# robotvisionmu/DenseMonoSLAM

Measured on AMD Instinct MI355X. Metric: frames/sec ICP+RGB+fusion @640x480, higher is better.
Workload: dtype f32; 1 GPU; TUM fr1/desk-like 640x480 full 3-level ICP+RGB tracking (SO3 + {10,5,4} GN iterations) + surfel index-map fusion; synthetic box-room RGB-D stream, loop closure off (--o), NID keyframing off (--nkf); cameras_per_gpu=1, n_pred=2, n_pred_project_passes=1, surfels_per_map=246557, surfels_total=246557, exchange=none (1 camera)

## Files before the change

densemonoslam_amd/csrc/exact_arith.hpp:

```cpp
#pragma once
#include <hip/hip_runtime.h>

namespace dms {
namespace exact {

struct Divisor {
  float d, y;
};

__device__ __forceinline__ Divisor divisor(float d) { return Divisor{d, 1.0f / d}; }

__device__ __forceinline__ float div(float a, const Divisor& c) {
  float q = a * c.y;
  float r = __builtin_fmaf(-c.d, q, a);
  q = __builtin_fmaf(r, c.y, q);
  r = __builtin_fmaf(-c.d, q, a);
  return __builtin_fmaf(r, c.y, q);
}

__device__ __forceinline__ float sqrt_normal(float a) {
  const float s = __builtin_amdgcn_sqrtf(a);
  const float sd = __uint_as_float(__float_as_uint(s) - 1u), su = __uint_as_float(__float_as_uint(s) + 1u);
  const float ed = __builtin_fmaf(-sd, s, a), eu = __builtin_fmaf(-su, s, a);
  float o = ed <= 0.f ? sd : s;
  o = eu > 0.f ? su : o;
  return o;
}

__device__ __forceinline__ float rcp_1_4(float s) {
  const float y0 = __builtin_amdgcn_rcpf(s);
  const float e = __builtin_fmaf(-s, y0, 1.0f);
  return __builtin_fmaf(e, y0, y0);
}

__device__ __forceinline__ Divisor divisor_1_4(float s) { return Divisor{s, rcp_1_4(s)}; }

}
}
```

densemonoslam_amd/csrc/fusion_fuse.hip:

```cpp
#include "scan.hpp"
#include "smallmath.hpp"
#include <utility>

#include "surfel.hpp"

namespace dms {

struct FuseArgs {
  const dms_pose_block* pose;
  const uchar4* rgba;
  const float* dr;
  const float* drf;
  const unsigned* index;
  const float4* vertConf;
  const float4* normRad;
  int cols, rows, slot_h;
  float cx, cy, icx, icy;
  float maxDepth, timef, weighting;
  const float* weighting_dev;
  int time, timeIdx;
  int transposed;
  int xcd;
};

__device__ __forceinline__ f3 dv_vertex(const float* depth, int cols, int sx, int sy, float x, float y, float cx, float cy, float icx,
                                        float icy) {
  const float z = depth[(size_t)sy * cols + sx];
  return mk3(((x - cx) * z) * icx, ((y - cy) * z) * icy, z);
}

__device__ __forceinline__ f3 dv_normal(const float* depth, int cols, int rows, const f3& vPosition, float tx, float ty, float x, float y,
                                        float cx, float cy, float icx, float icy) {
  const float colsf = (float)cols, rowsf = (float)rows;
  const int sx = texel(tx, colsf, cols), sy = texel(ty, rowsf, rows);
  const int sxf = texel(tx + (1.0f / colsf), colsf, cols), sxb = texel(tx - (1.0f / colsf), colsf, cols);
  const int syf = texel(ty + (1.0f / rowsf), rowsf, rows), syb = texel(ty - (1.0f / rowsf), rowsf, rows);
  const f3 xf = dv_vertex(depth, cols, sxf, sy, x + 1.f, y, cx, cy, icx, icy);
  const f3 xb = dv_vertex(depth, cols, sxb, sy, x - 1.f, y, cx, cy, icx, icy);
  const f3 yf = dv_vertex(depth, cols, sx, syf, x, y + 1.f, cx, cy, icx, icy);
  const f3 yb = dv_vertex(depth, cols, sx, syb, x, y - 1.f, cx, cy, icx, icy);
  const f3 del_x = mk3(((xb.x + vPosition.x) / 2.f) - ((xf.x + vPosition.x) / 2.f), ((xb.y + vPosition.y) / 2.f) - ((xf.y + vPosition.y) / 2.f),
                       ((xb.z + vPosition.z) / 2.f) - ((xf.z + vPosition.z) / 2.f));
  const f3 del_y = mk3(((yb.x + vPosition.x) / 2.f) - ((yf.x + vPosition.x) / 2.f), ((yb.y + vPosition.y) / 2.f) - ((yf.y + vPosition.y) / 2.f),
                       ((yb.z + vPosition.z) / 2.f) - ((yf.z + vPosition.z) / 2.f));
  return normalized3(cross3(del_x, del_y));
}

__device__ __forceinline__ float angle_between(const f3& a, const f3& b) {
  return det_acosf(dot3(a, b) / (length3(a) * length3(b)));
}

__global__ __launch_bounds__(256) void k_fuse_associate(FuseArgs a, float4* __restrict__ slot_pos, float4* __restrict__ slot_col,
                                                        float4* __restrict__ slot_nrm, unsigned* __restrict__ slot_best,
                                                        unsigned char* __restrict__ slot_flag, unsigned* __restrict__ winner, int slot_w) {
  const int tiles_j = (a.slot_h + 7) >> 3;
  const int t = xcd_block(blockIdx.x, gridDim.x, a.xcd) * (blockDim.x >> 6) + (threadIdx.x >> 6);
  const int ti = t / tiles_j, tj = t - ti * tiles_j;
  const int lane = threadIdx.x & 63, quad = lane >> 2, sub = lane & 3;
  const int i = ti * 2 + (quad >> 3);
  const int j = tj * 8 + (quad & 7);
  if (i >= slot_w || j >= a.slot_h) return;
  const int slot = i * a.slot_h + j;
  const int par = ((a.time % 2) + 2) % 2;
  const int px = 2 * i + par, py = 2 * j + par;
  unsigned char flag = 0;
  if (px < a.cols && py < a.rows) {
    const float colsf = (float)a.cols, rowsf = (float)a.rows;
    const float tx = uv_coord(px, a.cols), ty = uv_coord(py, a.rows);
    const float x = tx * colsf, y = ty * rowsf;
    const int sx = texel(tx, colsf, a.cols), sy = texel(ty, rowsf, a.rows);
    const f3 vPosLocal = dv_vertex(a.dr, a.cols, sx, sy, x, y, a.cx, a.cy, a.icx, a.icy);
    bool ok = ((int)x % 2 == (int)a.timef % 2) && ((int)y % 2 == (int)a.timef % 2);
    if (ok) {
      const int sxb = texel(tx - (1.0f / colsf), colsf, a.cols), sxf = texel(tx + (1.0f / colsf), colsf, a.cols);
      const int syb = texel(ty - (1.0f / rowsf), rowsf, a.rows), syf = texel(ty + (1.0f / rowsf), rowsf, a.rows);
      ok = !(a.dr[(size_t)sy * a.cols + sxb] == 0.f) && !(a.dr[(size_t)syb * a.cols + sx] == 0.f) &&
           !(a.dr[(size_t)sy * a.cols + sxf] == 0.f) && !(a.dr[(size_t)syf * a.cols + sx] == 0.f);
    }
    ok = ok && vPosLocal.z > 0.f && vPosLocal.z <= a.maxDepth;
    const float weighting = a.weighting_dev ? *a.weighting_dev : a.weighting;
    ok = ok && !(weighting < 0.f);
    if (ok) {
      const float* P = a.pose->pose;
      const f3 vPos = xform_point(P, vPosLocal);
      const f3 vPos_f = dv_vertex(a.drf, a.cols, sx, sy, x, y, a.cx, a.cy, a.icx, a.icy);
      const uchar4 c = a.rgba[(size_t)sy * a.cols + sx];
      const f3 vNormLocal = dv_normal(a.drf, a.cols, a.rows, vPos_f, tx, ty, x, y, a.cx, a.cy, a.icx, a.icy);
      const f3 nG = xform_dir(P, vNormLocal);
      const float rad = surfel_radius(vPos_f.z, vNormLocal.z, a.icx, a.icy);
      const float conf = surfel_confidence(x, y, a.cx, a.cy, weighting);

      int counter = 0;
      unsigned best = 0u;
      const float scale = 1.0f;
      const float indexXStep = (1.0f / (colsf * scale)) * 0.5f;
      const float indexYStep = (1.0f / (rowsf * scale)) * 0.5f;
      float bestDist = 1000.f;
      const float windowMultiplier = 2.f;
      const float xl = (x - a.cx) * a.icx;
      const float yl = (y - a.cy) * a.icy;
      const float lambda = sqrtf((xl * xl + yl * yl) + 1.f);
      const f3 ray = mk3(xl, yl, 1.f);
      const float ray_len = length3(ray);
      const float x_lo = tx - ((scale * indexXStep) * windowMultiplier), x_hi = tx + ((scale * indexXStep) * windowMultiplier);
      const float y_lo = ty - ((scale * indexYStep) * windowMultiplier), y_hi = ty + ((scale * indexYStep) * windowMultiplier);
      const AxisTaps tx_ = axis_taps(x_lo, x_hi, indexXStep, colsf, a.cols);
      const AxisTaps ty_ = axis_taps(y_lo, y_hi, indexYStep, rowsf, a.rows);
      const int txs_s = sub == 0 ? tx_.t0 : sub == 1 ? tx_.t1 : sub == 2 ? tx_.t2 : tx_.t3;
      const int mxs_s = sub == 0 ? tx_.m0 : sub == 1 ? tx_.m1 : sub == 2 ? tx_.m2 : tx_.m3;
      const int tys[4] = {ty_.t0, ty_.t1, ty_.t2, ty_.t3}, mys[4] = {ty_.m0, ty_.m1, ty_.m2, ty_.m3};
      size_t q[4];
      bool used[4];
      unsigned cur[4];
      float4 vcs[4], nrs[4];
#pragma unroll
      for (int jj = 0; jj < 4; ++jj) {
        const bool u = mxs_s != 0 && mys[jj] != 0;
        const int ux = u ? txs_s : 0, uy = u ? tys[jj] : 0;
        used[jj] = u;
        q[jj] = a.transposed ? (size_t)ux * a.rows + uy : (size_t)uy * a.cols + ux;
      }
#pragma unroll
      for (int jj = 0; jj < 4; ++jj) {
        cur[jj] = a.index[q[jj]];
        vcs[jj] = a.vertConf[q[jj]];
        nrs[jj] = a.normRad[q[jj]];
      }
      int order = 64;
#pragma unroll
      for (int jj = 0; jj < 4; ++jj) {
        const unsigned current = cur[jj];
        if (used[jj] && current > 0u) {
          const float4 vc = vcs[jj];
          if (fabsf((vc.z * lambda) - (vPosLocal.z * lambda)) < 0.05f) {
            const float dist = length3(cross3(ray, mk3(vc.x, vc.y, vc.z))) / ray_len;
            const float4 nr = nrs[jj];
            if (dist < bestDist && (fabsf(nr.z) < 0.75f || fabsf(angle_between(mk3(nr.x, nr.y, nr.z), vNormLocal)) < 0.5f)) {
              counter++;
              bestDist = dist;
              best = current;
              order = sub * 4 + jj;
            }
          }
        }
      }
#pragma unroll
      for (int m = 1; m < 4; m <<= 1) {
        const float od = __shfl_xor(bestDist, m, 64);
        const int oo = __shfl_xor(order, m, 64);
        const unsigned ob = __shfl_xor(best, m, 64);
        counter += __shfl_xor(counter, m, 64);
        if (od < bestDist || (od == bestDist && oo < order)) {
          bestDist = od;
          order = oo;
          best = ob;
        }
      }
      flag = counter > 0 ? 1 : 2;
      if (sub == 0) {
        slot_pos[slot] = make_float4(vPos.x, vPos.y, vPos.z, conf);
        slot_col[slot] = make_float4(encode_color_bytes(c.x, c.y, c.z), 0.f, a.timef, flag == 1 ? -1.f : -2.f);
        slot_nrm[slot] = make_float4(nG.x, nG.y, nG.z, rad);
        slot_best[slot] = best;
        if (flag == 1) atomicMin(winner + best, (unsigned)slot);
      }
    }
  }
  if (sub == 0) slot_flag[slot] = flag;
}

__global__ __launch_bounds__(256) void k_fuse_update(int nslots, const float4* __restrict__ slot_pos, const float4* __restrict__ slot_col,
                                                     const float4* __restrict__ slot_nrm, const unsigned* __restrict__ slot_best,
                                                     const unsigned char* __restrict__ slot_flag, unsigned* __restrict__ winner,
                                                     SurfelPlanes sp, size_t cap, int time, int timeIdx) {
  const int slot = blockIdx.x * blockDim.x + threadIdx.x;
  if (slot >= nslots || slot_flag[slot] != 1) return;
  const unsigned id = slot_best[slot];
  if (winner[id] != (unsigned)slot) return;
  winner[id] = kEmptyWinner;
  fuse_update_apply(id, (unsigned)slot, slot_pos, slot_col, slot_nrm, sp, cap, time, timeIdx);
}

struct CleanArgs {
  const dms_pose_block* pose;
  const unsigned* index;
  const float4* vertConf;
  const float4* colorTime;
  const float* depth_synth;
  int cols, rows;
  float cx, cy, fx, fy;
  float confThreshold, maxDepth;
  int time, timeIdx, timeDelta, isFern;
  int nodes;
  const float* node_table;
  int nslots;
  int transposed;
  int suffix;
  int num_sensors;
  int planes;
};

struct F4 {
  float x, y, z, w;
};
__device__ __forceinline__ F4 ld4(const float4* p) {
  const float4 t = *p;
  F4 r;
  r.x = t.x;
  r.y = t.y;
  r.z = t.z;
  r.w = t.w;
  return r;
}
__device__ __forceinline__ float4 to4(const F4& v) { return make_float4(v.x, v.y, v.z, v.w); }
struct CleanElem {
  F4 pos, col, nrm;
  float times[DMS_MAX_SENSORS];
  float vt;
};

__device__ __forceinline__ bool clean_load(unsigned e, unsigned M, const SurfelPlanes& sp, size_t cap, const float4* slot_pos,
                                           const float4* slot_col, const float4* slot_nrm, const unsigned char* slot_flag, int nslots,
                                           int timeIdx, int planes, CleanElem& o) {
  if (e < M) {
    o.pos = ld4(sp.pos + e);
    o.col = ld4(sp.col + e);
    o.nrm = ld4(sp.nrm + e);
#pragma unroll
    for (int s = 0; s < DMS_MAX_SENSORS; ++s) o.times[s] = s < planes ? sp.times[(size_t)s * cap + e] : -3.f;
    o.vt = sp.times[(size_t)timeIdx * cap + e];
    return true;
  }
  const unsigned slot = e - M;
  if ((int)slot >= nslots || slot_flag[slot] == 0) return false;
  o.pos = ld4(slot_pos + slot);
  o.col = ld4(slot_col + slot);
  o.nrm = ld4(slot_nrm + slot);
#pragma unroll
  for (int s = 0; s < DMS_MAX_SENSORS; ++s) o.times[s] = (s == timeIdx) ? o.col.w : -3.f;
  o.vt = o.col.w;
  return true;
}

__device__ __forceinline__ int clean_test(const CleanArgs& a, const CleanElem& v) {
  int test = 1;
  const float* Tinv = a.pose->t_inv;
  const f3 localPos = xform_point(Tinv, mk3(v.pos.x, v.pos.y, v.pos.z));
  const float x = ((a.fx * localPos.x) / localPos.z) + a.cx;
  const float y = ((a.fy * localPos.y) / localPos.z) + a.cy;
  const f3 localNorm = normalized3(xform_dir(Tinv, mk3(v.nrm.x, v.nrm.y, v.nrm.z)));
  const float colsf = (float)a.cols, rowsf = (float)a.rows;
  const float scale = 1.0f;
  const float indexXStep = (1.0f / (colsf * scale)) * 0.5f;
  const float indexYStep = (1.0f / (rowsf * scale)) * 0.5f;
  const float windowMultiplier = 2.f;
  int count = 0, zCount = 0;
  const float vt = v.vt;
  if ((float)a.time - vt < (float)a.timeDelta && localPos.z > 0.f && x > 0.f && y > 0.f && x < colsf && y < rowsf) {
    const float xc = x / colsf, yc = y / rowsf;
    const float x_lo = xc - ((scale * indexXStep) * windowMultiplier), x_hi = xc + ((scale * indexXStep) * windowMultiplier);
    const float y_lo = yc - ((scale * indexYStep) * windowMultiplier), y_hi = yc + ((scale * indexYStep) * windowMultiplier);
    const AxisTaps tx_ = axis_taps(x_lo, x_hi, indexXStep, colsf, a.cols);
    const AxisTaps ty_ = axis_taps(y_lo, y_hi, indexYStep, rowsf, a.rows);
    const int txs[4] = {tx_.t0, tx_.t1, tx_.t2, tx_.t3}, mxs[4] = {tx_.m0, tx_.m1, tx_.m2, tx_.m3};
    const int tys[4] = {ty_.t0, ty_.t1, ty_.t2, ty_.t3}, mys[4] = {ty_.m0, ty_.m1, ty_.m2, ty_.m3};
#pragma unroll
    for (int i = 0; i < 4; ++i) {
      if (mxs[i] != 0) {
        float4 vcs[4];
        unsigned qs[4];
        int mult[4];
#pragma unroll
        for (int j = 0; j < 4; ++j) {
          mult[j] = mxs[i] * mys[j];
          const int uy = mult[j] ? tys[j] : 0;
          qs[j] = a.transposed ? (unsigned)txs[i] * (unsigned)a.rows + (unsigned)uy : (unsigned)uy * (unsigned)a.cols + (unsigned)txs[i];
          vcs[j] = a.vertConf[qs[j]];
        }
#pragma unroll
        for (int j = 0; j < 4; ++j) {
          const int m = mult[j];
          const float4 vc = vcs[j];
          if (m != 0 && vc.w > a.confThreshold && vc.z > localPos.z) {
            const unsigned cur = a.index[qs[j]];
            const float2 ct = *reinterpret_cast<const float2*>(reinterpret_cast<const float*>(&a.colorTime[qs[j]]) + 2);
            if (cur > 0u) {
              const float ctz = ct.x, ctw = ct.y;
              const float dx = vc.x - localPos.x, dy = vc.y - localPos.y;
              if (ctz < v.col.z && vc.z - localPos.z < 0.01f && sqrtf(dx * dx + dy * dy) < v.nrm.w * 1.4f) count += m;
              if (ctw == (float)a.time && vc.z - localPos.z > 0.01f && fabsf(localNorm.z) > 0.85f) zCount += m;
            }
          }
        }
      }
    }
  }
  if (count > 8 || zCount > 4) test = 0;
  const float vt2 = (vt == -2.f) ? (float)a.time : vt;
  int unHealthy = 0;
#pragma unroll
  for (int s = 0; s < DMS_MAX_SENSORS; ++s) {
    const float ts = (s == a.timeIdx) ? vt2 : v.times[s];
    if (s < a.num_sensors && (ts == -1.f || (((float)a.time - ts) > 20.f && v.pos.w < a.confThreshold))) unHealthy++;
  }
  if (unHealthy == a.num_sensors) test = 0;
  if (vt2 > 0.f && (float)a.time - vt2 > (float)a.timeDelta) test = 1;
  return test;
}

__global__ __launch_bounds__(256) void k_clean_flags(CleanArgs a, SurfelPlanes sp, size_t cap, const unsigned* __restrict__ d_count,
                                                     const float4* slot_pos, const float4* slot_col, const float4* slot_nrm,
                                                     const unsigned char* slot_flag, unsigned char* __restrict__ keep,
                                                     unsigned* __restrict__ block_count, unsigned* __restrict__ first_touched) {
  const unsigned M = d_count[0];
  const unsigned total = M + (unsigned)a.nslots;
  const unsigned base = blockIdx.x * kScanChunk;
  if (first_touched && blockIdx.x == 0 && threadIdx.x == 0) *first_touched = 0xFFFFFFFFu;
  unsigned cnt = 0;
  if (base < total) {
    for (int k = 0; k < kScanChunk / 256; ++k) {
      const unsigned e = base + k * 256 + threadIdx.x;
      unsigned char f = 0;
      if (e < total) {
        CleanElem v;
        if (a.suffix && e < M) {
          v.pos = ld4(sp.pos + e);
#pragma unroll
          for (int s = 0; s < DMS_MAX_SENSORS; ++s) v.times[s] = s < a.planes ? sp.times[(size_t)s * cap + e] : -3.f;
          v.vt = sp.times[(size_t)a.timeIdx * cap + e];
          const f3 lp = xform_point(a.pose->t_inv, mk3(v.pos.x, v.pos.y, v.pos.z));
          const float x = ((a.fx * lp.x) / lp.z) + a.cx, y = ((a.fy * lp.y) / lp.z) + a.cy;
          const bool windowed = (float)a.time - v.vt < (float)a.timeDelta && lp.z > 0.f && x > 0.f && y > 0.f && x < (float)a.cols &&
                                y < (float)a.rows;
          const F4 zero = {0.f, 0.f, 0.f, 0.f};
          v.col = windowed ? ld4(sp.col + e) : zero;
          v.nrm = windowed ? ld4(sp.nrm + e) : zero;
          f = (unsigned char)clean_test(a, v);
        } else if (clean_load(e, M, sp, cap, slot_pos, slot_col, slot_nrm, slot_flag, a.nslots, a.timeIdx, a.planes, v)) {
          f = (unsigned char)clean_test(a, v);
        }
        keep[e] = f;
      }
      cnt += f;
    }
  }
  const unsigned tot = block_sum_u32(cnt);
  if (threadIdx.x == 0) block_count[blockIdx.x] = tot;
}

__device__ __forceinline__ f3 node_pos(const float* nt, int j) { return mk3(nt[j * 16 + 0], nt[j * 16 + 1], nt[j * 16 + 2]); }
// ... 209 lines not shown
          v.col.w = (float)a.time;
          v.vt = (float)a.time;
        }
        out.pos[dst] = to4(v.pos);
        out.col[dst] = to4(v.col);
        out.nrm[dst] = to4(v.nrm);
#pragma unroll
        for (int s = 0; s < DMS_MAX_SENSORS; ++s)
          if (s < a.planes) out.times[(size_t)s * cap + dst] = (s == a.timeIdx) ? v.vt : v.times[s];
      }
    }
    if (e >= M && e < total) slot_flag[e - M] = 0;
  }
}

static bool dense_img(const dms_image2d& im, size_t elem, int w, int h) {
  return im.data && im.cols == w && im.rows == h && im.pitch == (size_t)w * elem;
}

int model_fuse(dms_model* m, const dms_pose_block* pose, int time, int timeIdx, const dms_image2d* rgba, const dms_image2d* dr,
               const dms_image2d* drf, const dms_indexmap_out* im, const dms_camera* cam, float depthCutoff, float weighting,
               const float* weighting_dev, int transposed, hipStream_t s, int defer_update) {
  DMS_REQUIRE(m && pose && rgba && dr && drf && im && cam, "null argument");
  DMS_REQUIRE(!m->pending_update, "a deferred update pass is still pending (index_map applies it)");
  DMS_REQUIRE(timeIdx >= 0 && timeIdx < DMS_MAX_SENSORS, "timeIdx out of range");
  if (m->live_planes < timeIdx + 1) m->live_planes = timeIdx + 1;
  const int W = m->width, H = m->height;
  DMS_REQUIRE(dense_img(*rgba, 4, W, H) && dense_img(*dr, 4, W, H) && dense_img(*drf, 4, W, H) && dense_img(im->index, 4, W, H) &&
                  dense_img(im->vertConf, 16, W, H) && dense_img(im->normRad, 16, W, H),
              "dense W×H images required");
  FuseArgs a;
  a.xcd = xcd_remap_enabled();
  a.pose = pose;
  a.rgba = (const uchar4*)rgba->data;
  a.dr = (const float*)dr->data;
  a.drf = (const float*)drf->data;
  a.index = (const unsigned*)im->index.data;
  a.vertConf = (const float4*)im->vertConf.data;
  a.normRad = (const float4*)im->normRad.data;
  a.cols = W;
  a.rows = H;
  a.slot_h = m->slot_h;
  a.cx = cam->cx;
  a.cy = cam->cy;
  a.icx = (float)(1.0 / (double)cam->fx);
  a.icy = (float)(1.0 / (double)cam->fy);
  a.maxDepth = depthCutoff;
  a.timef = (float)time;
  a.weighting = weighting;
  a.weighting_dev = weighting_dev;
  a.time = time;
  a.timeIdx = timeIdx;
  a.transposed = transposed ? 1 : 0;
  const int slot_w = (W + 1) / 2;
  const int tiles = ((m->slot_h + 7) / 8) * ((slot_w + 1) / 2);
  dim3 b(256), g((tiles + 3) / 4);
  hipLaunchKernelGGL(k_fuse_associate, g, b, 0, s, a, m->slot_pos, m->slot_col, m->slot_nrm, m->slot_best, m->slot_flag, m->winner, slot_w);
  DMS_CHECK_LAUNCH();
  if (defer_update) {
    m->pending_update = true;
    m->pending_time = time;
    m->pending_timeIdx = timeIdx;
  } else {
    hipLaunchKernelGGL(k_fuse_update, dim3((m->slots + 255) / 256), dim3(256), 0, s, m->slots, m->slot_pos, m->slot_col, m->slot_nrm,
                       m->slot_best, m->slot_flag, m->winner, m->buf[m->cur], m->cap, time, timeIdx);
    DMS_CHECK_LAUNCH();
  }
  m->version += 1;
  return DMS_OK;
}

int model_flush_pending(dms_model* m, hipStream_t s) {
  if (!m || !m->pending_update) return DMS_OK;
  m->pending_update = false;
  hipLaunchKernelGGL(k_fuse_update, dim3((m->slots + 255) / 256), dim3(256), 0, s, m->slots, m->slot_pos, m->slot_col, m->slot_nrm, m->slot_best,
                     m->slot_flag, m->winner, m->buf[m->cur], m->cap, m->pending_time, m->pending_timeIdx);
  DMS_CHECK_LAUNCH();
  return DMS_OK;
}

int model_clean(dms_model* m, const dms_pose_block* pose, int time, int timeIdx, const dms_indexmap_out* im, const dms_image2d* depth_synth,
                const dms_camera* cam, float confThreshold, const float* graph_host, int graph_nodes, int timeDelta, float maxDepth,
                int isFern, int transposed, unsigned* count_out2, hipStream_t s) {
  DMS_REQUIRE(m && !m->pending_update, "a deferred update pass is still pending (index_map applies it)");
  DMS_REQUIRE(m && pose && im && cam, "null argument");
  DMS_REQUIRE(timeIdx >= 0 && timeIdx < DMS_MAX_SENSORS, "timeIdx out of range");
  const int W = m->width, H = m->height;
  DMS_REQUIRE(dense_img(im->index, 4, W, H) && dense_img(im->vertConf, 16, W, H) && dense_img(im->colorTime, 16, W, H),
              "dense W×H index-map images required");
  if (graph_nodes >= m->max_nodes) {
    set_error("dms_model_clean: %d deformation nodes exceed the limit %d", graph_nodes, m->max_nodes);
    return DMS_ERR_CAPACITY;
  }
  if (graph_nodes > 0) {
    DMS_REQUIRE(graph_host, "null graph");
    DMS_HIP(hipMemcpyAsync(m->nodes, graph_host, (size_t)graph_nodes * 16 * sizeof(float), hipMemcpyHostToDevice, s));
  }
  CleanArgs a;
  a.pose = pose;
  a.index = (const unsigned*)im->index.data;
  a.vertConf = (const float4*)im->vertConf.data;
  a.colorTime = (const float4*)im->colorTime.data;
  a.depth_synth = (depth_synth && depth_synth->data) ? (const float*)depth_synth->data : nullptr;
  a.cols = W;
  a.rows = H;
  a.cx = cam->cx;
  a.cy = cam->cy;
  a.fx = cam->fx;
  a.fy = cam->fy;
  a.confThreshold = confThreshold;
  a.maxDepth = maxDepth;
  a.time = time;
  a.timeIdx = timeIdx;
  a.timeDelta = timeDelta;
  a.isFern = isFern;
  a.nodes = graph_nodes;
  a.node_table = m->nodes;
  a.nslots = m->slots;
  a.transposed = transposed ? 1 : 0;
  const size_t upper = m->count_upper + (size_t)m->slots;
  const int nb = (int)((upper + kScanChunk - 1) / kScanChunk);
  const bool suffix = graph_nodes == 0 && upper >= m->clean_suffix_min;
  a.suffix = suffix ? 1 : 0;
  a.num_sensors = m->num_sensors;
  if (m->live_planes < timeIdx + 1) m->live_planes = timeIdx + 1;
  static const bool all_planes = getenv("DMS_CLEAN_ALL_PLANES") != nullptr;
  a.planes = all_planes ? DMS_MAX_SENSORS : m->live_planes;
  const SurfelPlanes src = m->buf[m->cur], dst = m->buf[m->cur ^ 1];
  hipLaunchKernelGGL(k_clean_flags, dim3(nb), dim3(256), 0, s, a, src, m->cap, m->d_count, m->slot_pos, m->slot_col, m->slot_nrm,
                     m->slot_flag, m->keep, m->block_count, suffix ? m->clean_first : (unsigned*)nullptr);
  DMS_CHECK_LAUNCH();
  static const int inline_max = getenv("DMS_CLEAN_INLINE_SCAN_MAX") ? atoi(getenv("DMS_CLEAN_INLINE_SCAN_MAX")) : 2048;
  const bool inline_scan = nb <= inline_max && !suffix;
  if (!inline_scan) {
    hipLaunchKernelGGL(k_scan_blocks_par, dim3((nb + 1023) / 1024), dim3(1024), 0, s, m->block_count, m->block_offset, nb, m->d_count_alt,
                       (unsigned)m->cap, count_out2, suffix ? m->clean_first : (unsigned*)nullptr, m->d_count, (unsigned)kScanChunk);
    DMS_CHECK_LAUNCH();
  }
  const int suffix_grid = nb < 2048 ? nb : 2048;
  if (suffix)
    hipLaunchKernelGGL(k_clean_scatter_suffix, dim3(suffix_grid), dim3(256), 0, s, a, src, m->cap, m->d_count, m->slot_pos, m->slot_col,
                       m->slot_nrm, m->slot_flag, m->keep, m->block_offset, dst, m->clean_first);
  else
    hipLaunchKernelGGL(k_clean_scatter, dim3(nb), dim3(256), 0, s, a, src, m->cap, m->d_count, m->slot_pos, m->slot_col, m->slot_nrm,
                       m->slot_flag, m->keep, m->block_offset, dst, inline_scan ? m->block_count : (const unsigned*)nullptr, m->d_count_alt,
                       count_out2);
  DMS_CHECK_LAUNCH();
  if (suffix) {
    hipLaunchKernelGGL(k_clean_copy_back, dim3(suffix_grid), dim3(256), 0, s, dst, src, m->cap, m->d_count_alt, m->clean_first, a.planes);
    DMS_CHECK_LAUNCH();
  }
  std::swap(m->d_count, m->d_count_alt);
  if (!suffix) m->cur ^= 1;
  m->count_upper = upper < m->cap ? upper : m->cap;
  m->version += 1;
  return DMS_OK;
}

}
```

densemonoslam_amd/csrc/fusion_map.hip:

```cpp
#include <vector>

#include "exact_arith.hpp"
#include "scan.hpp"
#include "smallmath.hpp"
#include "surfel.hpp"
#include "fill.hpp"
#include "internal.hpp"
#include "track_init.hpp"

namespace dms {
int model_flush_pending(dms_model* m, hipStream_t s);

static size_t up256(size_t v) { return (v + 255) / 256 * 256; }

struct ModelCarver {
  char* base = nullptr;
  size_t off = 0;
  template <typename T>
  T* take(size_t n) {
    off = up256(off);
    T* p = base ? (T*)(base + off) : nullptr;
    off += n * sizeof(T);
    return p;
  }
// ... 8 lines not shown
  }
  m->d_count = c.take<unsigned>(8);
  m->d_count_alt = m->d_count ? m->d_count + 4 : nullptr;
  m->slot_pos = c.take<float4>(m->slots);
  m->slot_col = c.take<float4>(m->slots);
  m->slot_nrm = c.take<float4>(m->slots);
  m->slot_best = c.take<unsigned>(m->slots);
  m->slot_flag = c.take<unsigned char>(m->slots);
  m->winner = c.take<unsigned>(m->cap);
  const size_t total = m->cap + (size_t)m->width * m->height;
  m->keep = c.take<unsigned char>(total);
  m->block_count = c.take<unsigned>(total / kScanChunk + 2);
  m->block_offset = c.take<unsigned>(total / kScanChunk + 2);
  m->clean_first = c.take<unsigned>(4);
  m->nodes = c.take<float>((size_t)m->max_nodes * 16);
}

__global__ void k_fill_u32(unsigned* p, size_t n, unsigned v) {
  for (size_t i = blockIdx.x * (size_t)blockDim.x + threadIdx.x; i < n; i += (size_t)blockDim.x * gridDim.x) p[i] = v;
}

}

using namespace dms;

extern "C" {

int dms_model_create(dms_model** out, size_t capacity, int width, int height) {
  DMS_REQUIRE(out && width >= 16 && height >= 16, "bad argument");
  dms_model* m = new dms_model();
  m->cap = capacity ? capacity : (size_t)5700 * 5700;
  m->width = width;
  m->height = height;
  m->slot_h = (height + 1) / 2;
  m->slots = ((width + 1) / 2) * m->slot_h;
  ModelCarver sz;
  model_layout(m, sz);
  m->arena_bytes = up256(sz.off);
  hipError_t e = hipMalloc((void**)&m->arena, m->arena_bytes);
  if (e != hipSuccess) {
    delete m;
    return hip_fail(e, "hipMalloc(model)", __FILE__, __LINE__);
  }
  ModelCarver c;
  c.base = m->arena;
  model_layout(m, c);
  e = hipHostMalloc((void**)&m->h_count, 8 * sizeof(unsigned), hipHostMallocDefault);
  if (e != hipSuccess) {
    (void)hipFree(m->arena);
    delete m;
    return hip_fail(e, "hipHostMalloc", __FILE__, __LINE__);
  }
  DMS_HIP(hipMemset(m->d_count, 0, 8 * sizeof(unsigned)));
  hipLaunchKernelGGL(k_fill_u32, dim3(1024), dim3(256), 0, 0, m->winner, m->cap, kEmptyWinner);
  DMS_CHECK_LAUNCH();
  for (int b = 0; b < 2; ++b) {
    hipLaunchKernelGGL(k_fill_u32, dim3(2048), dim3(256), 0, 0, (unsigned*)m->buf[b].times, m->cap * DMS_MAX_SENSORS, 0xC0400000u);
    DMS_CHECK_LAUNCH();
  }
  DMS_HIP(hipDeviceSynchronize());
  m->count_upper = 0;
  if (const char* smin = getenv("DMS_CLEAN_SUFFIX_MIN")) m->clean_suffix_min = (size_t)atoll(smin);
  *out = m;
  return DMS_OK;
}

int dms_model_set_num_sensors(dms_model* m, int num_sensors) {
  DMS_REQUIRE(m, "null argument");
  DMS_REQUIRE(num_sensors >= 1 && num_sensors <= DMS_MAX_SENSORS, "num_sensors out of range");
  m->num_sensors = num_sensors;
  return DMS_OK;
}

int dms_model_set_clean_suffix_min(dms_model* m, size_t surfels) {
  DMS_REQUIRE(m, "null argument");
  m->clean_suffix_min = surfels;
  return DMS_OK;
}

int dms_model_destroy(dms_model* m) {
  if (!m) return DMS_OK;
  if (m->arena) (void)hipFree(m->arena);
  if (m->h_count) (void)hipHostFree(m->h_count);
  delete m;
  return DMS_OK;
}

size_t dms_model_capacity(dms_model* m) { return m ? m->cap : 0; }
size_t dms_model_count_bound(dms_model* m) { return m ? m->count_upper : 0; }

int dms_model_count(dms_model* m, unsigned int* count, dms_stream s) {
  DMS_REQUIRE(m && count, "null argument");
  DMS_HIP(hipMemcpyAsync(m->h_count, m->d_count, sizeof(unsigned), hipMemcpyDeviceToHost, (hipStream_t)s));
  DMS_HIP(hipStreamSynchronize((hipStream_t)s));
  *count = m->h_count[0];
  m->count_upper = *count;
  return DMS_OK;
}

static int model_download_planes(dms_model* m, unsigned n, std::vector<float4>& pos, std::vector<float4>& col, std::vector<float4>& nrm,
                                 std::vector<float>& times, hipStream_t s) {
  const SurfelPlanes& b = m->buf[m->cur];
  pos.resize(n);
  col.resize(n);
  nrm.resize(n);
  times.resize((size_t)n * DMS_MAX_SENSORS);
// ... 1044 lines not shown
```

densemonoslam_amd/csrc/selftest.hip:

```cpp
#include "exact_arith.hpp"
#include "internal.hpp"

namespace dms {

template <int WHAT>
__global__ __launch_bounds__(256) void k_exact_check(unsigned first, unsigned long long n, float d, unsigned long long* __restrict__ bad,
                                                     unsigned* __restrict__ first_bad) {
  const unsigned long long t = (unsigned long long)blockIdx.x * blockDim.x + threadIdx.x;
  const exact::Divisor c = exact::divisor(d);
  unsigned long long mine = 0;
  unsigned which = 0;
  for (unsigned long long i = t * 256ull; i < t * 256ull + 256ull && i < n; ++i) {
    const unsigned bits = first + (unsigned)i;
    const float a = __uint_as_float(bits);
    float want, got;
    if (WHAT == 0) {
      want = sqrtf(a);
      got = exact::sqrt_normal(a);
    } else if (WHAT == 1) {
      want = 1.0f / a;
      got = exact::rcp_1_4(a);
    } else {
      if (!(fabsf(a) <= 3.4028234e38f)) continue;
      if (a != 0.f && fabsf(a) < 1.2621774e-29f) continue;
      want = a / d;
      if (a != 0.f && !(fabsf(want) >= 1.2621774e-29f && fabsf(want) <= 3.4028234e38f)) continue;
      got = exact::div(a, c);
      if (want == 0.f && got == 0.f) continue;
    }
    if (__float_as_uint(want) != __float_as_uint(got)) {
      mine += 1;
      which = bits;
    }
  }
  if (mine) {
    atomicAdd(bad, mine);
    atomicMax(first_bad, which);
  }
}

}

using namespace dms;

extern "C" int dms_exact_arith_selftest(int what, float d, unsigned long long* mismatches, unsigned* first_bad) {
  DMS_REQUIRE(mismatches && what >= 0 && what <= 2, "bad argument");
  DMS_REQUIRE(what != 2 || (d == d && fabsf(d) >= 1.17549435e-38f && fabsf(d) <= 3.4028234e38f), "the divisor must be a normal number");
  unsigned first = 0;
  unsigned long long n = 0;
  if (what == 0) {
    first = 0x0F800000u;
    n = 0x7F800000ull - first;
  } else if (what == 1) {
    first = 0x3F800000u;
    n = 0x40800000ull - first;
  } else {
    first = 0u;
    n = 1ull << 32;
  }
  unsigned long long* d_bad = nullptr;
  DMS_HIP(hipMalloc((void**)&d_bad, 16));
  DMS_HIP(hipMemset(d_bad, 0, 16));
  unsigned* d_first = (unsigned*)(d_bad + 1);
  const unsigned long long threads = (n + 255ull) / 256ull;
  const unsigned blocks = (unsigned)((threads + 255ull) / 256ull);
  if (what == 0)
    hipLaunchKernelGGL(k_exact_check<0>, dim3(blocks), dim3(256), 0, 0, first, n, d, d_bad, d_first);
  else if (what == 1)
    hipLaunchKernelGGL(k_exact_check<1>, dim3(blocks), dim3(256), 0, 0, first, n, d, d_bad, d_first);
  else
    hipLaunchKernelGGL(k_exact_check<2>, dim3(blocks), dim3(256), 0, 0, first, n, d, d_bad, d_first);
  hipError_t e = hipGetLastError();
  unsigned long long host[2] = {0, 0};
  if (e == hipSuccess) e = hipMemcpy(host, d_bad, 16, hipMemcpyDeviceToHost);
  (void)hipFree(d_bad);
  if (e != hipSuccess) return hip_fail(e, "exact-arithmetic self-test", __FILE__, __LINE__);
  *mismatches = host[0];
  if (first_bad) *first_bad = (unsigned)host[1];
  return DMS_OK;
}
```

densemonoslam_amd/csrc/surfel.hpp:

```cpp
#pragma once
#include "common.hpp"
#include "detmath.hpp"
#include "../../include/dmslam_fusion.h"

namespace dms {

struct SurfelPlanes {
  float4* pos;
  float4* col;
  float4* nrm;
  float* times;
};

constexpr unsigned kEmptyWinner = 0xFFFFFFFFu;
constexpr unsigned long long kZClear = (0xFFFFFFull << 32) | 0xFFFFFFFFull;
constexpr int kScanChunk = 256;

__host__ __device__ __forceinline__ int texel(float u, float n_f, int n) {
  int i = (int)floorf(u * n_f);
  if (i < 0) i = 0;
  if (i > n - 1) i = n - 1;
  return i;
}
__host__ __device__ __forceinline__ unsigned depth24(float zw) {
  if (!(zw >= 0.f)) return 0xFFFFFFFFu;
  if (zw > 1.f) return 0xFFFFFFFFu;
  return (unsigned)(int)rint((double)zw * 16777215.0);
}

__host__ __device__ __forceinline__ f3 xform_point(const float* M, const f3& p) {
  return mk3(((M[0] * p.x + M[1] * p.y) + M[2] * p.z) + M[3], ((M[4] * p.x + M[5] * p.y) + M[6] * p.z) + M[7],
             ((M[8] * p.x + M[9] * p.y) + M[10] * p.z) + M[11]);
}
__host__ __device__ __forceinline__ f3 xform_dir(const float* M, const f3& v) {
  return mk3((M[0] * v.x + M[1] * v.y) + M[2] * v.z, (M[4] * v.x + M[5] * v.y) + M[6] * v.z,
             (M[8] * v.x + M[9] * v.y) + M[10] * v.z);
}
__host__ __device__ __forceinline__ float length3(const f3& a) { return sqrtf(dot3(a, a)); }

__host__ __device__ __forceinline__ float surfel_radius(float depth, float norm_z, float cam_z, float cam_w) {
  const float meanFocal = ((1.0f / fabsf(cam_z)) + (1.0f / fabsf(cam_w))) / 2.0f;
  const float sqrt2 = 1.41421356237f;
  const float radius = (depth / meanFocal) * sqrt2;
  float radius_n = radius;
  radius_n = radius_n / fabsf(norm_z);
  radius_n = fminf(2.0f * radius, radius_n);
  return radius_n;
}
__host__ __device__ __forceinline__ float surfel_confidence(float x, float y, float cx, float cy, float weighting) {
  const float maxRadDist = 400.f;
  const float twoSigmaSquared = 0.72f;
  const float px = x - cx, py = y - cy;
  const float radialDist = sqrtf(px * px + py * py) / maxRadDist;
  return det_expf((-(radialDist * radialDist) / twoSigmaSquared)) * weighting;
}
__host__ __device__ __forceinline__ float encode_color_bytes(unsigned r, unsigned g, unsigned b) {
  return (float)(int)((((r << 8) + g) << 8) + b);
}
__host__ __device__ __forceinline__ float encode_color(float cx, float cy, float cz) {
  int rgb = (int)roundf(cx * 255.0f);
  rgb = (rgb << 8) + (int)roundf(cy * 255.0f);
  rgb = (rgb << 8) + (int)roundf(cz * 255.0f);
  return (float)rgb;
}
__host__ __device__ __forceinline__ f3 decode_color(float c) {
  const int ci = (int)c;
  return mk3((float)((ci >> 16) & 0xFF) / 255.0f, (float)((ci >> 8) & 0xFF) / 255.0f, (float)(ci & 0xFF) / 255.0f);
}

struct AxisTaps {
  int t0, t1, t2, t3;
  int m0, m1, m2, m3;
};
__device__ __forceinline__ AxisTaps axis_taps(float lo, float hi, float step, float nf, int n) {
  AxisTaps a = {-1, -1, -1, -1, 0, 0, 0, 0};
  int k = -1, last = -0x7fffffff;
  for (float w = lo; w < hi; w += step) {
    const int u = texel(w, nf, n);
    if (u != last) {
      ++k;
      last = u;
      if (k == 0) a.t0 = u;
      else if (k == 1) a.t1 = u;
      else if (k == 2) a.t2 = u;
      else a.t3 = u;
    }
    if (k == 0) a.m0++;
    else if (k == 1) a.m1++;
    else if (k == 2) a.m2++;
    else a.m3++;
  }
  return a;
}
template <class F>
__device__ __forceinline__ void for_taps(const AxisTaps& a, F f) {
  if (a.m0) f(a.t0, a.m0);
  if (a.m1) f(a.t1, a.m1);
  if (a.m2) f(a.t2, a.m2);
  if (a.m3) f(a.t3, a.m3);
}

__host__ __device__ __forceinline__ float uv_coord(int i, int n) {
  return (float)((double)((float)i / (float)n) + 1.0 / (double)(2.0f * (float)n));
}

__device__ __forceinline__ f3 fb_vertex(const float* depth, int cols, int sx, int sy, float x, float y, float cx, float cy, float ifx,
                                        float ify) {
  const float z = depth[(size_t)sy * cols + sx];
  return mk3(((x - cx) * z) * ifx, ((y - cy) * z) * ify, z);
}

__device__ __forceinline__ f3 fb_normal(const float* depth, int cols, int rows, const f3& vPosition, float tx, float ty, float x, float y,
                                        float cx, float cy, float ifx, float ify) {
  const float colsf = (float)cols, rowsf = (float)rows;
  const int sx = texel(tx, colsf, cols), sy = texel(ty, rowsf, rows);
  const int sxf = texel(tx + (1.0f / colsf), colsf, cols), sxb = texel(tx - (1.0f / colsf), colsf, cols);
  const int syf = texel(ty + (1.0f / rowsf), rowsf, rows), syb = texel(ty - (1.0f / rowsf), rowsf, rows);
  const f3 xf = fb_vertex(depth, cols, sxf, sy, x + 1.f, y, cx, cy, ifx, ify);
  const f3 xb = fb_vertex(depth, cols, sxb, sy, x - 1.f, y, cx, cy, ifx, ify);
  const f3 yf = fb_vertex(depth, cols, sx, syf, x, y + 1.f, cx, cy, ifx, ify);
  const f3 yb = fb_vertex(depth, cols, sx, syb, x, y - 1.f, cx, cy, ifx, ify);
  const f3 del_x = mk3(((xb.x + vPosition.x) / 2.f) - ((xf.x + vPosition.x) / 2.f), ((xb.y + vPosition.y) / 2.f) - ((xf.y + vPosition.y) / 2.f),
                       ((xb.z + vPosition.z) / 2.f) - ((xf.z + vPosition.z) / 2.f));
  const f3 del_y = mk3(((yb.x + vPosition.x) / 2.f) - ((yf.x + vPosition.x) / 2.f), ((yb.y + vPosition.y) / 2.f) - ((yf.y + vPosition.y) / 2.f),
                       ((yb.z + vPosition.z) / 2.f) - ((yf.z + vPosition.z) / 2.f));
  return normalized3(cross3(del_x, del_y));
}

__device__ __forceinline__ void fuse_update_apply(unsigned id, unsigned slot, const float4* __restrict__ slot_pos, const float4* __restrict__ slot_col,
                                                  const float4* __restrict__ slot_nrm, const SurfelPlanes& sp, size_t cap, int time, int timeIdx) {
  const float4 newPos = slot_pos[slot], newColor = slot_col[slot], newNorm = slot_nrm[slot];
  const float4 vPosition = sp.pos[id], vColor = sp.col[id], vNormRad = sp.nrm[id];
  const float c_k = vPosition.w;
  const float av = newPos.w;
  if (newNorm.w < (1.0f + 0.5f) * vNormRad.w) {
    const float wsum = c_k + av;
    sp.pos[id] = make_float4(((c_k * vPosition.x) + (av * newPos.x)) / wsum, ((c_k * vPosition.y) + (av * newPos.y)) / wsum,
                             ((c_k * vPosition.z) + (av * newPos.z)) / wsum, wsum);
    const f3 oldCol = decode_color(vColor.x), newCol = decode_color(newColor.x);
    const float ar = ((c_k * oldCol.x) + (av * newCol.x)) / wsum, ag = ((c_k * oldCol.y) + (av * newCol.y)) / wsum,
                ab = ((c_k * oldCol.z) + (av * newCol.z)) / wsum;
    sp.col[id] = make_float4(encode_color(ar, ag, ab), vColor.y, vColor.z, vColor.w);
    f3 n = mk3(((c_k * vNormRad.x) + (av * newNorm.x)) / wsum, ((c_k * vNormRad.y) + (av * newNorm.y)) / wsum,
               ((c_k * vNormRad.z) + (av * newNorm.z)) / wsum);
    const float r = ((c_k * vNormRad.w) + (av * newNorm.w)) / wsum;
    n = normalized3(n);
    sp.nrm[id] = make_float4(n.x, n.y, n.z, r);
  } else {
    sp.pos[id] = make_float4(vPosition.x, vPosition.y, vPosition.z, c_k + av);
  }
  sp.times[(size_t)timeIdx * cap + id] = (float)time;
}

}

struct dms_model {
  size_t cap = 0;
// ... 31 lines not shown
```

Before: 2754 frames/s.

## Hoist fusion constants to host and use exact-division and DPP quad shuffles

Per-launch constants (uv divisors, inverse sizes, index steps, mean focal) are now computed on the host and passed in, so each thread no longer recomputes them. Divisions and the sqrt comparison in the clean kernel are replaced by exactly rounded reciprocal-based division and a precomputed squared-bound test. Axis-tap computation is split across quad lanes and exchanged with DPP quad_perm instead of ds_swizzle/shfl. Vertex loads are skipped for masked taps, and the normal transform is deferred until it is actually needed. A self-test for the sqrt bound and a slot_flag memset are added, which adds code and relies on the bit-exact arithmetic being correct.

```diff
diff --git a/densemonoslam_amd/csrc/exact_arith.hpp b/densemonoslam_amd/csrc/exact_arith.hpp
--- a/densemonoslam_amd/csrc/exact_arith.hpp
+++ b/densemonoslam_amd/csrc/exact_arith.hpp
@@ -1,15 +1,51 @@
 #pragma once
+#include <cstdint>
+#include <cstring>
+#if defined(__HIPCC__)
 #include <hip/hip_runtime.h>
+#define DMS_EXACT_HD __host__ __device__ __forceinline__
+#else
+#define DMS_EXACT_HD inline
+#endif
 
 namespace dms {
 namespace exact {
+
+struct SqrtBound {
+  float b;
+};
+DMS_EXACT_HD SqrtBound sqrt_bound(float t) {
+  uint32_t u;
+  memcpy(&u, &t, 4);
+  uint32_t r;
+  if (!(t > 0.f)) {
+    r = 0xFF800000u;
+  } else if (u == 0x7F800000u) {
+    r = u;
+  } else {
+    const uint32_t ub = u - 1u;
+    float tb;
+    memcpy(&tb, &ub, 4);
+    const double m = ((double)tb + (double)t) * 0.5;
+    const double m2 = m * m;
+    const float f = (float)m2;
+    memcpy(&r, &f, 4);
+    if ((double)f < m2) r += 1u;
+  }
+  SqrtBound o;
+  memcpy(&o.b, &r, 4);
+  return o;
+}
+DMS_EXACT_HD bool sqrt_lt(float s, const SqrtBound& c) { return s >= 0.f && s < c.b; }
+DMS_EXACT_HD bool sqrt_lt(float s, float t) { return sqrt_lt(s, sqrt_bound(t)); }
 
 struct Divisor {
   float d, y;
 };
 
-__device__ __forceinline__ Divisor divisor(float d) { return Divisor{d, 1.0f / d}; }
+DMS_EXACT_HD Divisor divisor(float d) { return Divisor{d, 1.0f / d}; }
 
+#if defined(__HIPCC__)
 __device__ __forceinline__ float div(float a, const Divisor& c) {
   float q = a * c.y;
   float r = __builtin_fmaf(-c.d, q, a);
@@ -34,6 +70,7 @@
 }
 
 __device__ __forceinline__ Divisor divisor_1_4(float s) { return Divisor{s, rcp_1_4(s)}; }
+#endif
 
 }
 }
diff --git a/densemonoslam_amd/csrc/fusion_fuse.hip b/densemonoslam_amd/csrc/fusion_fuse.hip
--- a/densemonoslam_amd/csrc/fusion_fuse.hip
+++ b/densemonoslam_amd/csrc/fusion_fuse.hip
@@ -1,3 +1,4 @@
+#include "exact_arith.hpp"
 #include "scan.hpp"
 #include "smallmath.hpp"
 #include <utility>
@@ -21,7 +22,23 @@
   int time, timeIdx;
   int transposed;
   int xcd;
+  UvAxis uvx, uvy;
+  float inv_cols, inv_rows;
+  float indexXStep, indexYStep;
+  float meanFocal;
 };
+
+static void fuse_constants(FuseArgs& a) {
+  const float colsf = (float)a.cols, rowsf = (float)a.rows;
+  const float scale = 1.0f;
+  a.uvx = uv_axis(a.cols);
+  a.uvy = uv_axis(a.rows);
+  a.inv_cols = 1.0f / colsf;
+  a.inv_rows = 1.0f / rowsf;
+  a.indexXStep = (1.0f / (colsf * scale)) * 0.5f;
+  a.indexYStep = (1.0f / (rowsf * scale)) * 0.5f;
+  a.meanFocal = surfel_mean_focal(a.icx, a.icy);
+}
 
 __device__ __forceinline__ f3 dv_vertex(const float* depth, int cols, int sx, int sy, float x, float y, float cx, float cy, float icx,
                                         float icy) {
@@ -30,11 +47,11 @@
 }
 
 __device__ __forceinline__ f3 dv_normal(const float* depth, int cols, int rows, const f3& vPosition, float tx, float ty, float x, float y,
-                                        float cx, float cy, float icx, float icy) {
+                                        float cx, float cy, float icx, float icy, float inv_cols, float inv_rows) {
   const float colsf = (float)cols, rowsf = (float)rows;
   const int sx = texel(tx, colsf, cols), sy = texel(ty, rowsf, rows);
-  const int sxf = texel(tx + (1.0f / colsf), colsf, cols), sxb = texel(tx - (1.0f / colsf), colsf, cols);
-  const int syf = texel(ty + (1.0f / rowsf), rowsf, rows), syb = texel(ty - (1.0f / rowsf), rowsf, rows);
+  const int sxf = texel(tx + inv_cols, colsf, cols), sxb = texel(tx - inv_cols, colsf, cols);
+  const int syf = texel(ty + inv_rows, rowsf, rows), syb = texel(ty - inv_rows, rowsf, rows);
   const f3 xf = dv_vertex(depth, cols, sxf, sy, x + 1.f, y, cx, cy, icx, icy);
   const f3 xb = dv_vertex(depth, cols, sxb, sy, x - 1.f, y, cx, cy, icx, icy);
   const f3 yf = dv_vertex(depth, cols, sx, syf, x, y + 1.f, cx, cy, icx, icy);
@@ -44,6 +61,19 @@
   const f3 del_y = mk3(((yb.x + vPosition.x) / 2.f) - ((yf.x + vPosition.x) / 2.f), ((yb.y + vPosition.y) / 2.f) - ((yf.y + vPosition.y) / 2.f),
                        ((yb.z + vPosition.z) / 2.f) - ((yf.z + vPosition.z) / 2.f));
   return normalized3(cross3(del_x, del_y));
+}
+
+template <int P0, int P1, int P2, int P3>
+__device__ __forceinline__ int quad_perm(int v) {
+  return __builtin_amdgcn_mov_dpp(v, P0 | (P1 << 2) | (P2 << 4) | (P3 << 6), 0xF, 0xF, true);
+}
+template <int P0, int P1, int P2, int P3>
+__device__ __forceinline__ unsigned quad_perm(unsigned v) {
+  return (unsigned)quad_perm<P0, P1, P2, P3>((int)v);
+}
+template <int P0, int P1, int P2, int P3>
+__device__ __forceinline__ float quad_perm(float v) {
+  return __int_as_float(quad_perm<P0, P1, P2, P3>(__float_as_int(v)));
 }
 
 __device__ __forceinline__ float angle_between(const f3& a, const f3& b) {
@@ -66,14 +96,14 @@
   unsigned char flag = 0;
   if (px < a.cols && py < a.rows) {
     const float colsf = (float)a.cols, rowsf = (float)a.rows;
-    const float tx = uv_coord(px, a.cols), ty = uv_coord(py, a.rows);
+    const float tx = uv_coord(px, a.uvx), ty = uv_coord(py, a.uvy);
     const float x = tx * colsf, y = ty * rowsf;
     const int sx = texel(tx, colsf, a.cols), sy = texel(ty, rowsf, a.rows);
     const f3 vPosLocal = dv_vertex(a.dr, a.cols, sx, sy, x, y, a.cx, a.cy, a.icx, a.icy);
     bool ok = ((int)x % 2 == (int)a.timef % 2) && ((int)y % 2 == (int)a.timef % 2);
     if (ok) {
-      const int sxb = texel(tx - (1.0f / colsf), colsf, a.cols), sxf = texel(tx + (1.0f / colsf), colsf, a.cols);
-      const int syb = texel(ty - (1.0f / rowsf), rowsf, a.rows), syf = texel(ty + (1.0f / rowsf), rowsf, a.rows);
+      const int sxb = texel(tx - a.inv_cols, colsf, a.cols), sxf = texel(tx + a.inv_cols, colsf, a.cols);
+      const int syb = texel(ty - a.inv_rows, rowsf, a.rows), syf = texel(ty + a.inv_rows, rowsf, a.rows);
       ok = !(a.dr[(size_t)sy * a.cols + sxb] == 0.f) && !(a.dr[(size_t)syb * a.cols + sx] == 0.f) &&
            !(a.dr[(size_t)sy * a.cols + sxf] == 0.f) && !(a.dr[(size_t)syf * a.cols + sx] == 0.f);
     }
@@ -85,16 +115,15 @@
       const f3 vPos = xform_point(P, vPosLocal);
       const f3 vPos_f = dv_vertex(a.drf, a.cols, sx, sy, x, y, a.cx, a.cy, a.icx, a.icy);
       const uchar4 c = a.rgba[(size_t)sy * a.cols + sx];
-      const f3 vNormLocal = dv_normal(a.drf, a.cols, a.rows, vPos_f, tx, ty, x, y, a.cx, a.cy, a.icx, a.icy);
+      const f3 vNormLocal = dv_normal(a.drf, a.cols, a.rows, vPos_f, tx, ty, x, y, a.cx, a.cy, a.icx, a.icy, a.inv_cols, a.inv_rows);
       const f3 nG = xform_dir(P, vNormLocal);
-      const float rad = surfel_radius(vPos_f.z, vNormLocal.z, a.icx, a.icy);
+      const float rad = surfel_radius_mf(vPos_f.z, vNormLocal.z, a.meanFocal);
       const float conf = surfel_confidence(x, y, a.cx, a.cy, weighting);
 
       int counter = 0;
       unsigned best = 0u;
       const float scale = 1.0f;
-      const float indexXStep = (1.0f / (colsf * scale)) * 0.5f;
-      const float indexYStep = (1.0f / (rowsf * scale)) * 0.5f;
+      const float indexXStep = a.indexXStep, indexYStep = a.indexYStep;
       float bestDist = 1000.f;
       const float windowMultiplier = 2.f;
       const float xl = (x - a.cx) * a.icx;
@@ -104,10 +133,19 @@
       const float ray_len = length3(ray);
       const float x_lo = tx - ((scale * indexXStep) * windowMultiplier), x_hi = tx + ((scale * indexXStep) * windowMultiplier);
       const float y_lo = ty - ((scale * indexYStep) * windowMultiplier), y_hi = ty + ((scale * indexYStep) * windowMultiplier);
-      const AxisTaps tx_ = axis_taps(x_lo, x_hi, indexXStep, colsf, a.cols);
-      const AxisTaps ty_ = axis_taps(y_lo, y_hi, indexYStep, rowsf, a.rows);
-      const int txs_s = sub == 0 ? tx_.t0 : sub == 1 ? tx_.t1 : sub == 2 ? tx_.t2 : tx_.t3;
-      const int mxs_s = sub == 0 ? tx_.m0 : sub == 1 ? tx_.m1 : sub == 2 ? tx_.m2 : tx_.m3;
+      const bool oddLane = (sub & 1) != 0;
+      const AxisTaps tp = axis_taps(oddLane ? y_lo : x_lo, oddLane ? y_hi : x_hi, oddLane ? indexYStep : indexXStep, oddLane ? rowsf : colsf,
+                                    oddLane ? a.rows : a.cols);
+      AxisTaps ty_;
+      ty_.t0 = quad_perm<1, 1, 3, 3>(tp.t0), ty_.t1 = quad_perm<1, 1, 3, 3>(tp.t1), ty_.t2 = quad_perm<1, 1, 3, 3>(tp.t2);
+      ty_.t3 = quad_perm<1, 1, 3, 3>(tp.t3);
+      ty_.m0 = quad_perm<1, 1, 3, 3>(tp.m0), ty_.m1 = quad_perm<1, 1, 3, 3>(tp.m1), ty_.m2 = quad_perm<1, 1, 3, 3>(tp.m2);
+      ty_.m3 = quad_perm<1, 1, 3, 3>(tp.m3);
+      const bool hiPair = (sub & 2) != 0;
+      const int txE = quad_perm<0, 0, 2, 2>(hiPair ? tp.t2 : tp.t0), txO = quad_perm<0, 0, 2, 2>(hiPair ? tp.t3 : tp.t1);
+      const int mxE = quad_perm<0, 0, 2, 2>(hiPair ? tp.m2 : tp.m0), mxO = quad_perm<0, 0, 2, 2>(hiPair ? tp.m3 : tp.m1);
+      const int txs_s = oddLane ? txO : txE;
+      const int mxs_s = oddLane ? mxO : mxE;
       const int tys[4] = {ty_.t0, ty_.t1, ty_.t2, ty_.t3}, mys[4] = {ty_.m0, ty_.m1, ty_.m2, ty_.m3};
       size_t q[4];
       bool used[4];
@@ -146,10 +184,10 @@
       }
 #pragma unroll
       for (int m = 1; m < 4; m <<= 1) {
-        const float od = __shfl_xor(bestDist, m, 64);
-        const int oo = __shfl_xor(order, m, 64);
-        const unsigned ob = __shfl_xor(best, m, 64);
-        counter += __shfl_xor(counter, m, 64);
+        const float od = m == 1 ? quad_perm<1, 0, 3, 2>(bestDist) : quad_perm<2, 3, 0, 1>(bestDist);
+        const int oo = m == 1 ? quad_perm<1, 0, 3, 2>(order) : quad_perm<2, 3, 0, 1>(order);
+        const unsigned ob = m == 1 ? quad_perm<1, 0, 3, 2>(best) : quad_perm<2, 3, 0, 1>(best);
+        counter += m == 1 ? quad_perm<1, 0, 3, 2>(counter) : quad_perm<2, 3, 0, 1>(counter);
         if (od < bestDist || (od == bestDist && oo < order)) {
           bestDist = od;
           order = oo;
@@ -198,7 +236,18 @@
   int suffix;
   int num_sensors;
   int planes;
+  float indexXStep, indexYStep;
+  exact::Divisor colsD, rowsD;
 };
+
+static void clean_constants(CleanArgs& a) {
+  const float colsf = (float)a.cols, rowsf = (float)a.rows;
+  const float scale = 1.0f;
+  a.indexXStep = (1.0f / (colsf * scale)) * 0.5f;
+  a.indexYStep = (1.0f / (rowsf * scale)) * 0.5f;
+  a.colsD = exact::divisor(colsf);
+  a.rowsD = exact::divisor(rowsf);
+}
 
 struct F4 {
   float x, y, z, w;
@@ -248,16 +297,15 @@
   const f3 localPos = xform_point(Tinv, mk3(v.pos.x, v.pos.y, v.pos.z));
   const float x = ((a.fx * localPos.x) / localPos.z) + a.cx;
   const float y = ((a.fy * localPos.y) / localPos.z) + a.cy;
-  const f3 localNorm = normalized3(xform_dir(Tinv, mk3(v.nrm.x, v.nrm.y, v.nrm.z)));
   const float colsf = (float)a.cols, rowsf = (float)a.rows;
   const float scale = 1.0f;
-  const float indexXStep = (1.0f / (colsf * scale)) * 0.5f;
-  const float indexYStep = (1.0f / (rowsf * scale)) * 0.5f;
+  const float indexXStep = a.indexXStep, indexYStep = a.indexYStep;
   const float windowMultiplier = 2.f;
-  int count = 0, zCount = 0;
+  int count = 0, zSum = 0;
   const float vt = v.vt;
   if ((float)a.time - vt < (float)a.timeDelta && localPos.z > 0.f && x > 0.f && y > 0.f && x < colsf && y < rowsf) {
-    const float xc = x / colsf, yc = y / rowsf;
+    const float xc = exact::div(x, a.colsD), yc = exact::div(y, a.rowsD);
+    const exact::SqrtBound radBound = exact::sqrt_bound(v.nrm.w * 1.4f);
     const float x_lo = xc - ((scale * indexXStep) * windowMultiplier), x_hi = xc + ((scale * indexXStep) * windowMultiplier);
     const float y_lo = yc - ((scale * indexYStep) * windowMultiplier), y_hi = yc + ((scale * indexYStep) * windowMultiplier);
     const AxisTaps tx_ = axis_taps(x_lo, x_hi, indexXStep, colsf, a.cols);
@@ -273,9 +321,12 @@
 #pragma unroll
         for (int j = 0; j < 4; ++j) {
           mult[j] = mxs[i] * mys[j];
-          const int uy = mult[j] ? tys[j] : 0;
-          qs[j] = a.transposed ? (unsigned)txs[i] * (unsigned)a.rows + (unsigned)uy : (unsigned)uy * (unsigned)a.cols + (unsigned)txs[i];
-          vcs[j] = a.vertConf[qs[j]];
+          qs[j] = 0u;
+          vcs[j] = make_float4(0.f, 0.f, 0.f, 0.f);
+          if (mult[j] != 0) {
+            qs[j] = a.transposed ? (unsigned)txs[i] * (unsigned)a.rows + (unsigned)tys[j] : (unsigned)tys[j] * (unsigned)a.cols + (unsigned)txs[i];
+            vcs[j] = a.vertConf[qs[j]];
+          }
         }
 #pragma unroll
         for (int j = 0; j < 4; ++j) {
@@ -287,15 +338,20 @@
             if (cur > 0u) {
               const float ctz = ct.x, ctw = ct.y;
               const float dx = vc.x - localPos.x, dy = vc.y - localPos.y;
-              if (ctz < v.col.z && vc.z - localPos.z < 0.01f && sqrtf(dx * dx + dy * dy) < v.nrm.w * 1.4f) count += m;
-              if (ctw == (float)a.time && vc.z - localPos.z > 0.01f && fabsf(localNorm.z) > 0.85f) zCount += m;
+              if (ctz < v.col.z && vc.z - localPos.z < 0.01f && exact::sqrt_lt(dx * dx + dy * dy, radBound)) count += m;
+              if (ctw == (float)a.time && vc.z - localPos.z > 0.01f) zSum += m;
             }
           }
         }
       }
     }
   }
-  if (count > 8 || zCount > 4) test = 0;
+  if (count > 8) {
+    test = 0;
+  } else if (zSum > 4) {
+    const f3 localNorm = normalized3(xform_dir(Tinv, mk3(v.nrm.x, v.nrm.y, v.nrm.z)));
+    if (fabsf(localNorm.z) > 0.85f) test = 0;
+  }
   const float vt2 = (vt == -2.f) ? (float)a.time : vt;
   int unHealthy = 0;
 #pragma unroll
@@ -611,6 +667,7 @@
   a.time = time;
   a.timeIdx = timeIdx;
   a.transposed = transposed ? 1 : 0;
+  fuse_constants(a);
   const int slot_w = (W + 1) / 2;
   const int tiles = ((m->slot_h + 7) / 8) * ((slot_w + 1) / 2);
   dim3 b(256), g((tiles + 3) / 4);
@@ -677,6 +734,7 @@
   a.node_table = m->nodes;
   a.nslots = m->slots;
   a.transposed = transposed ? 1 : 0;
+  clean_constants(a);
   const size_t upper = m->count_upper + (size_t)m->slots;
   const int nb = (int)((upper + kScanChunk - 1) / kScanChunk);
   const bool suffix = graph_nodes == 0 && upper >= m->clean_suffix_min;
diff --git a/densemonoslam_amd/csrc/fusion_map.hip b/densemonoslam_amd/csrc/fusion_map.hip
--- a/densemonoslam_amd/csrc/fusion_map.hip
+++ b/densemonoslam_amd/csrc/fusion_map.hip
@@ -84,6 +84,7 @@
     return hip_fail(e, "hipHostMalloc", __FILE__, __LINE__);
   }
   DMS_HIP(hipMemset(m->d_count, 0, 8 * sizeof(unsigned)));
+  DMS_HIP(hipMemset(m->slot_flag, 0, (size_t)m->slots));
   hipLaunchKernelGGL(k_fill_u32, dim3(1024), dim3(256), 0, 0, m->winner, m->cap, kEmptyWinner);
   DMS_CHECK_LAUNCH();
   for (int b = 0; b < 2; ++b) {
diff --git a/densemonoslam_amd/csrc/selftest.hip b/densemonoslam_amd/csrc/selftest.hip
--- a/densemonoslam_amd/csrc/selftest.hip
+++ b/densemonoslam_amd/csrc/selftest.hip
@@ -39,12 +39,84 @@
   }
 }
 
+__global__ __launch_bounds__(256) void k_sqrt_lt_check(unsigned first, unsigned long long n, float d, int rad_form, unsigned long long* __restrict__ bad,
+                                                       unsigned* __restrict__ first_bad) {
+  const unsigned long long t0 = (unsigned long long)blockIdx.x * blockDim.x + threadIdx.x;
+  const float t = rad_form ? d * 1.4f : d;
+  const exact::SqrtBound c = exact::sqrt_bound(t);
+  unsigned long long mine = 0;
+  unsigned which = 0;
+  for (unsigned long long i = t0 * 256ull; i < t0 * 256ull + 256ull && i < n; ++i) {
+    const unsigned bits = first + (unsigned)i;
+    const float s = __uint_as_float(bits);
+    const bool want = sqrtf(s) < t;
+    const bool got = exact::sqrt_lt(s, c);
+    if (want != got) {
+      mine += 1;
+      which = bits;
+    }
+  }
+  if (mine) {
+    atomicAdd(bad, mine);
+    atomicMax(first_bad, which);
+  }
+}
+
 }
 
 using namespace dms;
 
+static int sqrt_lt_ranges(float t, unsigned (*out)[2]) {
+  int e2 = 127;
+  if (t > 0.f && t <= 3.4028234e38f) {
+    int e;
+    (void)frexpf(t, &e);
+    e2 = 2 * e - 2 + 127;
+  }
+  int lo = e2 - 8, hi = e2 + 8;
+  if (lo < 1) {
+    hi += 1 - lo;
+    lo = 1;
+  }
+  if (hi > 255) {
+    lo -= hi - 255;
+    hi = 255;
+  }
+  int k = 0;
+  out[k][0] = (unsigned)lo << 23, out[k++][1] = (unsigned)(hi - lo) << 23;
+  out[k][0] = 0u, out[k++][1] = 0x00800000u;
+  const unsigned few[] = {0x7F800000u, 0x7FC00000u, 0x7FFFFF00u, 0x80000000u, 0x80800000u, 0xBF800000u, 0xFF800000u, 0xFFC00000u};
+  for (unsigned f : few) out[k][0] = f, out[k++][1] = 0x100u;
+  return k;
+}
+
+static int sqrt_lt_selftest(int what, float d, unsigned long long* mismatches, unsigned* first_bad) {
+  const float t = what == 3 ? d * 1.4f : d;
+  unsigned ranges[16][2];
+  const int nr = sqrt_lt_ranges(t, ranges);
+  unsigned long long* d_bad = nullptr;
+  DMS_HIP(hipMalloc((void**)&d_bad, 16));
+  DMS_HIP(hipMemset(d_bad, 0, 16));
+  unsigned* d_first = (unsigned*)(d_bad + 1);
+  for (int r = 0; r < nr; ++r) {
+    const unsigned long long n = ranges[r][1];
+    const unsigned long long threads = (n + 255ull) / 256ull;
+    hipLaunchKernelGGL(k_sqrt_lt_check, dim3((unsigned)((threads + 255ull) / 256ull)), dim3(256), 0, 0, ranges[r][0], n, d, what == 3 ? 1 : 0, d_bad,
+                       d_first);
+  }
+  hipError_t e = hipGetLastError();
+  unsigned long long host[2] = {0, 0};
+  if (e == hipSuccess) e = hipMemcpy(host, d_bad, 16, hipMemcpyDeviceToHost);
+  (void)hipFree(d_bad);
+  if (e != hipSuccess) return hip_fail(e, "sqrt_lt self-test", __FILE__, __LINE__);
+  *mismatches = host[0];
+  if (first_bad) *first_bad = (unsigned)host[1];
+  return DMS_OK;
+}
+
 extern "C" int dms_exact_arith_selftest(int what, float d, unsigned long long* mismatches, unsigned* first_bad) {
-  DMS_REQUIRE(mismatches && what >= 0 && what <= 2, "bad argument");
+  DMS_REQUIRE(mismatches && what >= 0 && what <= 4, "bad argument");
+  if (what >= 3) return sqrt_lt_selftest(what, d, mismatches, first_bad);
   DMS_REQUIRE(what != 2 || (d == d && fabsf(d) >= 1.17549435e-38f && fabsf(d) <= 3.4028234e38f), "the divisor must be a normal number");
   unsigned first = 0;
   unsigned long long n = 0;
diff --git a/densemonoslam_amd/csrc/surfel.hpp b/densemonoslam_amd/csrc/surfel.hpp
--- a/densemonoslam_amd/csrc/surfel.hpp
+++ b/densemonoslam_amd/csrc/surfel.hpp
@@ -1,6 +1,7 @@
 #pragma once
 #include "common.hpp"
 #include "detmath.hpp"
+#include "exact_arith.hpp"
 #include "../../include/dmslam_fusion.h"
 
 namespace dms {
@@ -40,6 +41,17 @@
 
 __host__ __device__ __forceinline__ float surfel_radius(float depth, float norm_z, float cam_z, float cam_w) {
   const float meanFocal = ((1.0f / fabsf(cam_z)) + (1.0f / fabsf(cam_w))) / 2.0f;
+  const float sqrt2 = 1.41421356237f;
+  const float radius = (depth / meanFocal) * sqrt2;
+  float radius_n = radius;
+  radius_n = radius_n / fabsf(norm_z);
+  radius_n = fminf(2.0f * radius, radius_n);
+  return radius_n;
+}
+__host__ __device__ __forceinline__ float surfel_mean_focal(float cam_z, float cam_w) {
+  return ((1.0f / fabsf(cam_z)) + (1.0f / fabsf(cam_w))) / 2.0f;
+}
+__host__ __device__ __forceinline__ float surfel_radius_mf(float depth, float norm_z, float meanFocal) {
   const float sqrt2 = 1.41421356237f;
   const float radius = (depth / meanFocal) * sqrt2;
   float radius_n = radius;
@@ -103,6 +115,13 @@
 __host__ __device__ __forceinline__ float uv_coord(int i, int n) {
   return (float)((double)((float)i / (float)n) + 1.0 / (double)(2.0f * (float)n));
 }
+
+struct UvAxis {
+  exact::Divisor n;
+  double half;
+};
+inline UvAxis uv_axis(int n) { return UvAxis{exact::divisor((float)n), 1.0 / (double)(2.0f * (float)n)}; }
+__device__ __forceinline__ float uv_coord(int i, const UvAxis& c) { return (float)((double)exact::div((float)i, c.n) + c.half); }
 
 __device__ __forceinline__ f3 fb_vertex(const float* depth, int cols, int sx, int sy, float x, float y, float cx, float cy, float ifx,
                                         float ify) {
```

After: 2764 frames/s (median of 6 runs). Within noise of the previous version (+0.4%).
